# shenyunhang/JTSM

Measured on AMD Instinct MI355X. Metric: images/sec training, R50-FPN JTSM panoptic, 2x1024x1024, 1/2/4/8 GPU, higher is better.
Workload: dtype bf16x3; 1 GPU; BASELINE configs[2]: JTSM panoptic R50-FPN, 2 x 3x1024x1024 per GPU, 2000 proposals + 1024 superpixels per image; MIL + 4 OICR + 2 mask heads + sem-seg; fwd + bwd + gradient exchange + SGD; 100% of proposals jittered copies of 40 rectangles per image; global_batch=2, parallelism=dp1, foreground_rois_last_step=281

## Files before the change

### include/jtsm_hip.h

```cpp
#ifndef JTSM_HIP_H_
#define JTSM_HIP_H_

#include <stddef.h>
#include <stdint.h>

#ifdef __cplusplus
extern "C" {
#endif

#define JTSM_OK 0
#define JTSM_EINVAL (-1)
#define JTSM_ELAUNCH (-2)
#define JTSM_ENODEV (-3)

#define JTSM_NCHW 0
#define JTSM_NHWC 1

const char* jtsm_last_error(void);
const char* jtsm_version(void);
int jtsm_device_count(void);

void* jtsm_event_create(void);
int jtsm_event_record(void* event, void* stream);
int jtsm_event_elapsed_ms(void* start, void* stop, float* ms);
// ... 103 lines not shown
  int batch, in_h, in_w, in_c;
  int out_c;
  int kernel_h, kernel_w;
  int stride, pad, dilation;
} jtsm_conv_shape;

int jtsm_conv_out_size(const jtsm_conv_shape* s, int* out_h, int* out_w);
size_t jtsm_conv_workspace_bytes(const jtsm_conv_shape* s, int backward_data);
int jtsm_conv_plan(const jtsm_conv_shape* s, int role, int has_kscale, int* kernel, int* tile_m,
                   int* tile_n, int* splits);

int jtsm_conv2d_forward_f32(const float* x, const float* w, float* y, const jtsm_conv_shape* s,
                            const float* scale, const float* bias, const float* residual,
                            int relu, void* workspace, size_t workspace_bytes, void* stream);
int jtsm_conv2d_backward_data_f32(const float* dy, const float* w, float* dx,
                                  const jtsm_conv_shape* s, const float* kscale,
                                  const float* accumulate, const float* relu_mask, void* workspace,
                                  size_t workspace_bytes, void* stream);
int jtsm_conv2d_backward_weight_f32(const float* dy, const float* x, float* dw,
                                    const jtsm_conv_shape* s, const float* row_scale, int zero_dw,
                                    void* stream);

int jtsm_split_bf16_f32(const float* src, uint16_t* hi, uint16_t* lo, long n, void* stream);
int jtsm_split_bf16_paired_f32(const float* src, uint16_t* planes, long rows, int k, void* stream);
int jtsm_split_bf16_transposed_f32(const float* w, const float* row_scale, uint16_t* hi, uint16_t* lo,
                                   int out_c, int taps, int in_c, void* stream);
int jtsm_split_bf16_multi_f32(const void* table, int entries, long blocks, int transposed, void* stream);
int jtsm_conv_bf16x3_eligible(const jtsm_conv_shape* s, int role);
int jtsm_conv_bf16x3_plan(const jtsm_conv_shape* s, int role, int* wm, int* wn, int* tm, int* tn, int* nbuf,
                          int* splits);
int jtsm_conv2d_forward_bf16x3(const uint16_t* x_hi, const uint16_t* x_lo, const uint16_t* w_hi,
                               const uint16_t* w_lo, float* y, uint16_t* y_hi, uint16_t* y_lo,
                               const jtsm_conv_shape* s, const float* scale, const float* bias,
                               const float* residual, int relu, void* workspace, size_t workspace_bytes,
                               void* stream);
int jtsm_conv2d_backward_data_bf16x3(const uint16_t* dy_hi, const uint16_t* dy_lo, const uint16_t* wt_hi,
                                     const uint16_t* wt_lo, float* dx, uint16_t* dx_hi, uint16_t* dx_lo,
                                     const jtsm_conv_shape* s, const float* accumulate,
                                     const float* relu_mask, void* workspace, size_t workspace_bytes,
                                     void* stream);
size_t jtsm_conv_bf16x3_wgrad_workspace_bytes(const jtsm_conv_shape* s);
int jtsm_conv2d_backward_weight_bf16x3(const uint16_t* dy_hi, const uint16_t* dy_lo, const uint16_t* x_hi,
                                       const uint16_t* x_lo, float* dw, const jtsm_conv_shape* s,
                                       const float* row_scale, int zero_dw, void* workspace,
                                       size_t workspace_bytes, void* stream);

int jtsm_split_f16_f32(const float* src, uint16_t* h, long n, int shift, void* stream);
int jtsm_split_f16_transposed_f32(const float* w, const float* row_scale, uint16_t* h, int out_c, int taps, int in_c,
                                  void* stream);
int jtsm_conv2d_forward_f16(const uint16_t* x_h, const uint16_t* w_h, float* y, uint16_t* y_h,
                            const jtsm_conv_shape* s, const float* scale, const float* bias,
                            const float* residual, int relu, void* workspace, size_t workspace_bytes,
                            void* stream);
int jtsm_conv2d_backward_data_f16(const uint16_t* dy_h, const uint16_t* wt_h, float* dx, uint16_t* dx_h,
                                  const jtsm_conv_shape* s, const float* accumulate, const float* relu_mask,
                                  int grad_shift, void* workspace, size_t workspace_bytes, void* stream);
int jtsm_conv2d_backward_weight_f16(const uint16_t* dy_h, const uint16_t* x_h, float* dw, const jtsm_conv_shape* s,
                                    const float* row_scale, int zero_dw, int grad_shift, void* workspace,
                                    size_t workspace_bytes, void* stream);
int jtsm_conv_transpose2x2_forward_bf16x3(const uint16_t* x_hi, const uint16_t* x_lo, const uint16_t* wt_hi,
                                          const uint16_t* wt_lo, float* y, uint16_t* y_hi, uint16_t* y_lo, int batch,
                                          int h, int w, int in_c, int out_c, const float* bias, int relu, void* stream);
int jtsm_conv_transpose2x2_forward_f16(const uint16_t* x_h, const uint16_t* wt_h, float* y, uint16_t* y_h, int batch,
                                       int h, int w, int in_c, int out_c, const float* bias, int relu, void* stream);
size_t jtsm_conv_transpose2x2_workspace_bytes(int batch, int h, int w, int in_c, int out_c);
int jtsm_conv_transpose2x2_backward_data_bf16x3(const uint16_t* g_hi, const uint16_t* g_lo, const uint16_t* w_hi,
                                                const uint16_t* w_lo, float* dx, uint16_t* dx_hi, uint16_t* dx_lo,
                                                int batch, int h, int w, int in_c, int out_c, const float* relu_mask,
                                                const uint16_t* gate_plane, void* workspace, size_t workspace_bytes,
                                                void* stream);
int jtsm_conv_transpose2x2_backward_data_f16(const uint16_t* g_h, const uint16_t* w_h, float* dx, uint16_t* dx_h,
                                             int batch, int h, int w, int in_c, int out_c, const float* relu_mask,
                                             const uint16_t* gate_plane, int grad_shift, void* workspace,
                                             size_t workspace_bytes, void* stream);
int jtsm_conv2d_backward_data_ex_bf16x3(const uint16_t* dy_hi, const uint16_t* dy_lo, const uint16_t* wt_hi,
                                        const uint16_t* wt_lo, float* dx, uint16_t* dx_hi, uint16_t* dx_lo,
                                        const jtsm_conv_shape* s, const float* row_scale, const float* accumulate,
                                        const float* relu_mask, const uint16_t* gate_plane, void* workspace,
                                        size_t workspace_bytes, void* stream);
int jtsm_conv2d_backward_data_ex_f16(const uint16_t* dy_h, const uint16_t* wt_h, float* dx, uint16_t* dx_h,
                                     const jtsm_conv_shape* s, const float* row_scale, const float* accumulate,
                                     const float* relu_mask, const uint16_t* gate_plane, int grad_shift, void* workspace,
                                     size_t workspace_bytes, void* stream);

int jtsm_conv2d_forward_res16_f16(const uint16_t* x_h, const uint16_t* w_h, float* y, uint16_t* y_h,
                                  const jtsm_conv_shape* s, const float* scale, const float* bias,
                                  const uint16_t* residual_h, int relu, void* workspace, size_t workspace_bytes,
                                  void* stream);
int jtsm_conv2d_backward_data_acc16_f16(const uint16_t* dy_h, const uint16_t* wt_h, float* dx, uint16_t* dx_h,
                                        const jtsm_conv_shape* s, const float* row_scale, const uint16_t* accumulate_h,
                                        const uint16_t* gate_plane, int grad_shift, void* workspace,
                                        size_t workspace_bytes, void* stream);

int jtsm_conv_bf16x3_colsum_rows(const jtsm_conv_shape* s, int role);
int jtsm_conv2d_backward_data_colsum_bf16x3(const uint16_t* dy_hi, const uint16_t* dy_lo, const uint16_t* wt_hi,
                                            const uint16_t* wt_lo, float* dx, uint16_t* dx_hi, uint16_t* dx_lo,
                                            const jtsm_conv_shape* s, const float* row_scale, const float* accumulate,
                                            const float* relu_mask, const uint16_t* gate_plane, float* colsum,
                                            void* workspace, size_t workspace_bytes, void* stream);
int jtsm_conv2d_backward_data_colsum_f16(const uint16_t* dy_h, const uint16_t* wt_h, float* dx, uint16_t* dx_h,
                                         const jtsm_conv_shape* s, const float* row_scale, const float* accumulate,
                                         const float* relu_mask, const uint16_t* gate_plane, int grad_shift, float* colsum,
                                         void* workspace, size_t workspace_bytes, void* stream);
int jtsm_conv_transpose2x2_backward_data_colsum_bf16x3(const uint16_t* g_hi, const uint16_t* g_lo, const uint16_t* w_hi,
                                                       const uint16_t* w_lo, float* dx, uint16_t* dx_hi, uint16_t* dx_lo,
                                                       int batch, int h, int w, int in_c, int out_c,
                                                       const float* relu_mask, const uint16_t* gate_plane, float* colsum,
                                                       void* workspace, size_t workspace_bytes, void* stream);
int jtsm_conv_transpose2x2_backward_data_colsum_f16(const uint16_t* g_h, const uint16_t* w_h, float* dx, uint16_t* dx_h,
                                                    int batch, int h, int w, int in_c, int out_c, const float* relu_mask,
                                                    const uint16_t* gate_plane, int grad_shift, float* colsum,
                                                    void* workspace, size_t workspace_bytes, void* stream);
int jtsm_relu_backward_split_scaled_f32(const float* dy, const float* y, float scale, float* g, uint16_t* g_hi,
                                        uint16_t* g_lo, long n, int shift, void* stream);
int jtsm_split_rowscale_f32(const float* src, const float* row_scale, long rows, int cols, uint16_t* hi, uint16_t* lo,
                            int shift, void* stream);
int jtsm_dropout_split_f32(const float* x, float* y, uint16_t* y_hi, uint16_t* y_lo, long n, float p,
                           unsigned long long seed, void* stream);
int jtsm_channel_sum_planes(const uint16_t* hi, const uint16_t* lo, float* out, long rows, int C, int shift,
                            void* workspace, size_t workspace_bytes, void* stream);
int jtsm_channel_sum_planes_multi(const uint16_t* const* hi, const uint16_t* const* lo, float* const* outs,
                                  const long* rows, int count, int C, int shift, void* workspace,
                                  size_t workspace_bytes, void* stream);
size_t jtsm_conv_bf16x3_wgrad_bias_workspace_bytes(const jtsm_conv_shape* s);
int jtsm_conv2d_backward_weight_bias_bf16x3(const uint16_t* dy_hi, const uint16_t* dy_lo, const uint16_t* x_hi,
                                            const uint16_t* x_lo, float* dw, float* db, const jtsm_conv_shape* s,
                                            const float* row_scale, int zero_dw, void* workspace,
                                            size_t workspace_bytes, void* stream);
int jtsm_conv2d_backward_weight_bias_f16(const uint16_t* dy_h, const uint16_t* x_h, float* dw, float* db,
                                         const jtsm_conv_shape* s, const float* row_scale, int zero_dw, int grad_shift,
                                         void* workspace, size_t workspace_bytes, void* stream);
size_t jtsm_conv_bf16x3_wgrad_group_workspace_bytes(const jtsm_conv_shape* s, int n);
int jtsm_conv_bf16x3_wgrad_group_plan(const jtsm_conv_shape* s, int n, int* tile, int* splits);
int jtsm_conv2d_backward_weight_group_bf16x3(int n, const uint16_t* const* dy_hi, const uint16_t* const* dy_lo,
                                             const uint16_t* const* x_hi, const uint16_t* const* x_lo,
                                             float* const* dw, const float* const* row_scale,
                                             const jtsm_conv_shape* s, void* workspace, size_t workspace_bytes,
                                             void* stream);
int jtsm_conv2d_backward_weight_group_f16(int n, const uint16_t* const* dy_h, const uint16_t* const* x_h,
                                          float* const* dw, const float* const* row_scale, const jtsm_conv_shape* s,
                                          int grad_shift, void* workspace, size_t workspace_bytes, void* stream);
int jtsm_relu_backward_split_f16(const float* dy, const float* y, float* g, uint16_t* g_h, long n, int shift,
                                 void* stream);

int jtsm_relu_backward_split_f32(const float* dy, const float* y, float* g, uint16_t* g_hi, uint16_t* g_lo,
                                 long n, void* stream);
int jtsm_relu_backward_f32(const float* dy, const float* y, float* g, long n, void* stream);
int jtsm_channel_sum_f32(const float* g, float* out, long rows, int C, void* stream);
int jtsm_colsum_fold_f32(const float* const* parts, const int* rows, int n, int width, float* out, void* stream);
size_t jtsm_channel_sum_workspace_bytes(long rows, int C);
int jtsm_channel_sum_ws_f32(const float* g, float* out, long rows, int C, void* workspace, size_t workspace_bytes,
                            void* stream);
int jtsm_sgd_momentum_multi_f32(const void* table, int entries, long blocks, int first_step, void* stream);


int jtsm_maxpool3x3s2_forward_f32(const float* x, float* y, int N, int H, int W, int C, void* stream);
int jtsm_maxpool3x3s2_backward_f32(const float* x, const float* gy, float* gx, int N, int H, int W,
                                   int C, void* stream);
int jtsm_maxpool2x2_forward_f32(const float* x, float* y, int N, int H, int W, int C, int stride, void* stream);
int jtsm_maxpool2x2_backward_f32(const float* x, const float* gy, float* gx, int N, int H, int W, int C,
                                 int stride, void* stream);
int jtsm_upsample2_add_f32(const float* top, const float* lateral, float* out, uint16_t* out_hi, uint16_t* out_lo,
                           int N, int H, int W, int C, void* stream);
int jtsm_sum_tensors_f32(const float* const* inputs, int n, long numel, float* out, uint16_t* out_hi, uint16_t* out_lo,
                         void* stream);
int jtsm_sum2x2_f32(const float* g, float* out, int N, int Ht, int Wt, int C, void* stream);
int jtsm_subsample2_f32(const float* src, float* dst, int N, int H, int W, int C, int scatter,
                        void* stream);


size_t jtsm_mil_workspace_bytes(int nbags, int max_bag_rows, int nc);
int jtsm_mil_forward_f32(const float* cls_logits, const float* det_logits, int ld, int nc,
                         const int32_t* bag_offsets, int nbags, int max_bag_rows,
                         const float* labels, int mean_loss, float* scores, float* img_probs,
                         float* loss, void* workspace, void* stream);
int jtsm_mil_backward_f32(const float* cls_logits, const float* det_logits, int ld, int nc,
                          const int32_t* bag_offsets, int nbags, int max_bag_rows,
                          const float* upstream, float* d_cls, float* d_det, int ld_grad,
                          const void* workspace, void* stream);

size_t jtsm_oicr_workspace_bytes(void);
int jtsm_oicr_forward_f32(const float* cls_logits, int ld_cls, int num_cls, const float* box_deltas,
                          int ld_box, const int32_t* labels, const float* weights,
                          const float* proposals, const float* gt_boxes, int R, float* losses,
                          void* workspace, void* stream);
int jtsm_oicr_backward_f32(const float* cls_logits, int ld_cls, int num_cls, const float* box_deltas,
                           int ld_box, const int32_t* labels, const float* weights,
                           const float* proposals, const float* gt_boxes, int R, const float* losses,
                           const float* up_cls, const float* up_box, float* d_cls, int ld_dcls,
                           float* d_box, int ld_dbox, void* stream);


int jtsm_rect_mask_targets_f32(const float* rois, const float* rects, uint8_t* out, int N, int side, int H, int W,
                               float erode, void* stream);
int jtsm_sp_mask_targets_f32(const float* rois, const int32_t* oh_row, const int32_t* img_of, const int32_t* oh_labels,
                             int L, const int32_t* superpixels, uint8_t* out, int N, int side, int H, int W,
                             void* stream);
int jtsm_paste_crop_targets_f32(const float* probs, const float* rois, uint8_t* out, int N, int M, int side, int H,
                                int W, float threshold, void* stream);
int jtsm_near_targets_f32(const float* proposals, const int32_t* bag_offsets, int B, int R, const int32_t* labels,
                          int bg_label, const float* pgt_box, const int32_t* counts, int Gmax, int top_k,
                          int32_t* near_rows, int32_t* matched_near, void* stream);

int jtsm_pooler_rois_levels_f32(const float* const* boxes, const int* counts, int B, int min_level, int max_level,
                                float canonical_box_size, float canonical_level, float* rois, int32_t* level,
                                void* stream);
int jtsm_roi_scale_f32(const int32_t* argmax, int bins, int C, const float* const* objectness, const int* counts, int B,
                       float* out, void* stream);
size_t jtsm_image_labels_workspace_bytes(int B);
int jtsm_image_labels(const int64_t* const* gt_classes, const int* counts, int B, int num_classes, const void* sem_seg,
                      int sem_elem_bytes, long pixels, int num_stuff, int stuff_offset, float* oh_things,
                      int32_t* things_cls, int32_t* things_cnt, float* oh_stuff, int32_t* stuff_cls, int32_t* stuff_cnt,
                      void* workspace, void* stream);

int jtsm_fg_compact(const int32_t* labels, int bg_label, const int32_t* bag_offsets, int B, int R, const float* boxes,
                    const int32_t* matched, int32_t* fg_rows, float* fg_boxes, int64_t* fg_classes, int32_t* fg_img,
                    int32_t* fg_matched, float* fg_rois, int64_t* counts, void* stream);

size_t jtsm_mask_bce_workspace_bytes(void);
int jtsm_mask_bce_forward_f32(const float* logits, int ld, int num_classes, const int64_t* gt_classes,
                              const uint8_t* target, int N, int side, float* out, void* workspace,
                              void* stream);
int jtsm_mask_bce_backward_f32(const float* logits, int ld, int num_classes, const int64_t* gt_classes,
                               const uint8_t* target, int N, int side, const float* upstream,
                               float* dlogits, void* stream);


int jtsm_roi_align_forward_level_f32(const float* input, const float* rois,
                                     const int32_t* roi_level, int level, float* output, int B,
                                     int C, int H, int W, int M, float spatial_scale, int pooled_h,
                                     int pooled_w, int sampling_ratio, int aligned, void* stream);
int jtsm_roi_align_backward_level_f32(const float* grad, const float* rois,
                                      const int32_t* roi_level, int level, float* grad_input, int B,
                                      int C, int H, int W, int M, float spatial_scale, int pooled_h,
                                      int pooled_w, int sampling_ratio, int aligned, void* stream);
int jtsm_roi_align_rotated_forward_level_f32(const float* input, const float* rois, const int32_t* roi_level,
                                             int level, float* output, int B, int C, int H, int W, int M,
                                             float spatial_scale, int pooled_h, int pooled_w, int sampling_ratio,
                                             void* stream);
int jtsm_roi_align_rotated_backward_level_f32(const float* grad, const float* rois, const int32_t* roi_level,
                                              int level, float* grad_input, int B, int C, int H, int W, int M,
                                              float spatial_scale, int pooled_h, int pooled_w, int sampling_ratio,
                                              int accumulate, void* stream);
size_t jtsm_roi_align_backward_levels_workspace_bytes(const int* H, const int* W, int nlevels, int B, int C, int M);
int jtsm_roi_align_backward_levels_f32(const float* grad, const float* rois, const int32_t* roi_level,
                                       float* const* grad_inputs, const int* H, const int* W, const float* scales,
                                       int nlevels, int B, int C, int M, int pooled_h, int pooled_w, int sampling_ratio,
                                       int aligned, int accumulate, void* workspace, size_t workspace_bytes,
                                       void* stream);
int jtsm_moi_pool_forward_level_f32(const float* input, const float* rois, const int32_t* roi_level,
                                    int level, const int32_t* oh_labels, const int32_t* superpixels,
                                    float* output, int32_t* argmax, void* workspace, int B, int C,
                                    int H, int W, int M, int L, int Hs, int Ws, float spatial_scale,
                                    int pooled_h, int pooled_w, void* stream);
int jtsm_moi_pool_backward_level_f32(const float* grad, const float* rois, const int32_t* roi_level,
                                     int level, const int32_t* argmax, float* grad_input, int B, int C,
                                     int H, int W, int M, int pooled_h, int pooled_w, void* stream);


size_t jtsm_group_norm_workspace_bytes(int N, long HW, int C);
int jtsm_group_norm_forward_f32(const float* x, const float* gamma, const float* beta, float* y,
                                float* mean, float* rstd, void* workspace, int N, long HW, int C, int G,
                                float eps, int relu, void* stream);
int jtsm_group_norm_backward_f32(const float* x, const float* dy, const float* gamma, const float* beta,
                                 const float* mean, const float* rstd, float* dx, uint16_t* dx_hi,
                                 uint16_t* dx_lo, float* dgamma, float* dbeta, void* workspace, int N, long HW,
                                 int C, int G, int relu, void* stream);
int jtsm_upsample_bilinear2x_forward_f32(const float* x, float* y, uint16_t* y_hi, uint16_t* y_lo, int N, int H,
                                         int W, int C, void* stream);
int jtsm_upsample_bilinear2x_backward_f32(const float* gy, float* gx, int N, int H, int W, int C,
                                          void* stream);


size_t jtsm_semseg_ce_workspace_bytes(int N, int Hs, int Ws, int S);
int jtsm_semseg_ce_forward_f32(const float* logits, int ld, int C, const int64_t* target, float* out,
                               void* workspace, int N, int Hs, int Ws, int S, long ignore_index,
                               void* stream);
int jtsm_semseg_ce_backward_f32(const float* logits, int ld, int C, const int64_t* target,
                                const float* fwd_out, const float* upstream, float* dlogits,
                                const void* workspace, int N, int Hs, int Ws, int S, long ignore_index,
                                void* stream);


int jtsm_row_lse_f32(const float* logits, int ld, int ncls, int R, float* lse, void* stream);
int jtsm_mine_top1_f32(const float* scores, int ld, const float* lse, const float* proposals,
                       const float* deltas, int ld_deltas, const int32_t* bag_offsets,
                       const int32_t* classes, const int32_t* counts, int B, int Gmax,
                       const float* img_probs, int nprob, int32_t* out_idx, float* out_box,
                       float* out_score, float* out_weight, void* stream);
size_t jtsm_paint_sem_seg_workspace_bytes(int B);
int jtsm_paint_sem_seg(const float* boxes, const int32_t* classes, const float* scores, const int32_t* counts,
                       int B, int G, int class_base, int H, int W, float erode, int64_t* out, void* workspace,
                       void* stream);
int jtsm_paint_sem_seg_evidence(const int32_t* target_idx, const int32_t* bag_offsets, const int32_t* oh_labels, int L,
                                const int32_t* superpixels, const int32_t* classes, const float* scores,
                                const int32_t* counts, int B, int G, int class_base, int H, int W, int64_t* out,
                                void* workspace, void* stream);
int jtsm_match_label_f32(const float* proposals, const int32_t* bag_offsets, int B, int R,
                         const float* pgt_box, const int32_t* classes, const int32_t* counts,
                         const float* pgt_weight, const float* pgt_score, int Gmax, float iou_thresh,
                         int bg_label, int32_t* labels, int32_t* matched, float* gt_boxes,
                         float* gt_weights, float* gt_scores, void* stream);


int jtsm_oicr_predict_f32(const float* const* logits, const float* const* deltas, int heads, int R, int C1, int Kb,
                          const float* proposals, const float* weights , float scale_clamp, float* probs,
// ... 44 lines not shown
```

### jtsm_amd/build.py

```python
import argparse
import glob
import os
import subprocess
import sys
from concurrent.futures import ThreadPoolExecutor

HERE = os.path.dirname(os.path.abspath(__file__))
CSRC = os.path.join(HERE, "csrc")
OBJ = os.path.join(HERE, "lib", "obj")
LIB = os.path.join(HERE, "lib", "libjtsm_hip.so")
HIPCC = os.environ.get("HIPCC", "/opt/rocm/bin/hipcc")
FLAGS = ["--offload-arch=gfx950", "-O3", "-std=c++17", "-fPIC", "-Wall", "-Wno-unused-function",
         "-fno-gpu-rdc"] + os.environ.get("JTSM_EXTRA_HIPCC_FLAGS", "").split()
FILE_FLAGS = {"semseg_ops.hip": ["-fno-slp-vectorize"]}


def _stale(target, deps):
    if not os.path.isfile(target):
        return True
    t = os.path.getmtime(target)
    return any(os.path.getmtime(d) > t for d in deps)


def build(force=False, verbose=False, jobs=4):
    os.makedirs(OBJ, exist_ok=True)
    srcs = sorted(glob.glob(os.path.join(CSRC, "*.hip")))
    hdrs = sorted(glob.glob(os.path.join(CSRC, "*.h"))) + [
        os.path.join(HERE, "..", "include", "jtsm_hip.h")]
    todo, objs = [], []
    for s in srcs:
        o = os.path.join(OBJ, os.path.basename(s)[:-4] + ".o")
        objs.append(o)
        if force or _stale(o, [s, os.path.abspath(__file__)] + hdrs):
            todo.append((s, o))

    def cc(job):
        s, o = job
        cmd = [HIPCC] + FLAGS + FILE_FLAGS.get(os.path.basename(s), []) + ["-c", s, "-o", o]
        if verbose:
            print(" ".join(cmd), flush=True)
        r = subprocess.run(cmd, stdout=subprocess.PIPE, stderr=subprocess.STDOUT, text=True)
        return s, r.returncode, r.stdout

    if todo:
        with ThreadPoolExecutor(max_workers=jobs) as ex:
            for s, rc, out in ex.map(cc, todo):
                if out.strip() and (verbose or rc):
                    print(out, file=sys.stderr)
                if rc:
                    raise RuntimeError("hipcc failed on %s" % s)
    if todo or force or _stale(LIB, objs):
        cmd = [HIPCC, "--offload-arch=gfx950", "-shared", "-fPIC", "-o", LIB] + objs
        if verbose:
            print(" ".join(cmd), flush=True)
        subprocess.check_call(cmd)
    return LIB


if __name__ == "__main__":
    ap = argparse.ArgumentParser()
    ap.add_argument("--force", action="store_true")
    ap.add_argument("-v", "--verbose", action="store_true")
    a = ap.parse_args()
    print(build(force=a.force, verbose=a.verbose))
```

### jtsm_amd/layers/conv.py

```python
import ctypes as C
import os

import torch
from torch.autograd import Function
from torch.autograd.function import once_differentiable

from .. import _lib as L
from . import grad_fan

CL = torch.channels_last

LAUNCH_LOG = None
SEGMENT = "heads"


def set_segment(name):
    global SEGMENT
    SEGMENT = name


MATH = os.environ.get("JTSM_CONV_MATH", "bf16x3")
_MODES = ("f32", "bf16x3", "f16")
GRAD_SHIFT = int(os.environ.get("JTSM_F16_GRAD_SHIFT", "12"))
BIAS_IN_WGRAD = os.environ.get("JTSM_BIAS_IN_WGRAD", "1") != "0"


def planes_mode():
    return MATH != "f32"


def set_math(mode):
    global MATH
    if mode not in _MODES:
        raise ValueError("conv math must be one of %r, got %r" % (_MODES, mode))
    if mode != MATH:
        _drop_planes()
    MATH = mode


def _planes_buf(n, device):
    n8 = max((n + 7) // 8 * 8, 64)
    if MATH == "f16":
        return torch.empty(n8, dtype=torch.int16, device=device)
    return torch.empty(2 * n8, dtype=torch.int16, device=device)


def _hl(buf):
    if buf is None:
        return None, None
    p = buf.data_ptr()
    if MATH == "f16":
        return p, None
    if getattr(buf, "_paired", False):
        return p, p + 64
    return p, p + buf.numel()


W_PAIRED = os.environ.get("JTSM_W_PAIRED", "1") != "0"


def _paired_ok(w, transposed):
    if not W_PAIRED or MATH != "bf16x3" or w.numel() == 0:
        return 0
    k = w.numel() // w.shape[1 if transposed else 0]
    return k if k % 32 == 0 else 0


def _split(t, grad=False):
    flat = t.permute(0, 2, 3, 1) if t.dim() == 4 else t
    if not flat.is_contiguous():
        raise RuntimeError("split_bf16: tensor must be channels_last (4-d) or contiguous")
    buf = _planes_buf(t.numel(), t.device)
    hi, lo = _hl(buf)
    L.note_bytes((6.0 if MATH == "f16" else 8.0) * t.numel())
    if MATH == "f16":
        L.check(L.lib().jtsm_split_f16_f32(L.ptr(t), hi, t.numel(), GRAD_SHIFT if grad else 0, L.stream()), "split_f16")
        return buf
    L.check(L.lib().jtsm_split_bf16_f32(L.ptr(t), hi, lo, t.numel(), L.stream()), "split_bf16")
    return buf


def split_bf16(t):
    buf = _split(t)
    n8 = buf.numel() // 2
    return buf[:t.numel()], buf[n8:n8 + t.numel()]


def _split_paired(w):
    k = _paired_ok(w, False)
    buf = _planes_buf(w.numel(), w.device)
    buf._paired = True
    L.note_bytes(8.0 * w.numel())
    L.check(L.lib().jtsm_split_bf16_paired_f32(L.ptr(w), L.ptr(buf), w.numel() // k, k, L.stream()),
            "split_bf16_paired")
    return buf


def _split_transposed_into(buf, w, row_scale, paired=True):
    o, i, kh, kw = w.shape
    if paired and _paired_ok(w, True):
        buf._paired = True
    hi, lo = _hl(buf)
    if MATH == "f16":
        L.check(L.lib().jtsm_split_f16_transposed_f32(L.ptr(w), L.ptr(row_scale), hi, o, kh * kw, i, L.stream()),
                "split_f16_transposed")
    else:
        L.check(L.lib().jtsm_split_bf16_transposed_f32(L.ptr(w), L.ptr(row_scale), hi, lo, o, kh * kw, i, L.stream()),
                "split_bf16_transposed")
    return buf


def _split_transposed(w, row_scale=None, paired=True):
    return _split_transposed_into(_planes_buf(w.numel(), w.device), w, row_scale, paired)


def split_bf16_transposed(w, row_scale=None):
    buf = _split_transposed(w, row_scale, paired=False)
    n8 = buf.numel() // 2
    return buf[:w.numel()], buf[n8:n8 + w.numel()]


_PLANES = {}
_PLANES_MAX_BYTES = 16 << 30
_planes_bytes = 0


CLEAR_HOOKS = []


def planes_clear():
    global _planes_bytes
    _PLANES.clear()
    _planes_bytes = 0
    for hook in CLEAR_HOOKS:
        hook()
    refresh_weight_planes()


def _drop_planes():
    global _planes_bytes
    _PLANES.clear()
    _planes_bytes = 0
    _WPLANES.clear()
    _WTABLES.clear()


def planes_put(t, buf):
    global _planes_bytes
    if _planes_bytes > _PLANES_MAX_BYTES:
        _PLANES.clear()
        _planes_bytes = 0
    _PLANES[(t.data_ptr(), t.numel())] = (t.detach(), t._version, buf)
    _planes_bytes += 8 * t.numel()


def planes_forget(t):
    _PLANES.pop((t.data_ptr(), t.numel()), None)


def planes_of(t, grad=False):
    e = _PLANES.get((t.data_ptr(), t.numel()))
    if e is not None and e[1] == t._version:
        return e[2]
    buf = _split(t, grad)
    planes_put(t, buf)
    return buf


class _WEntry(object):
    __slots__ = ("w", "scale", "transposed", "buf", "version")


_WPLANES = {}
_WTABLES = {}


def _cacheable_weight(w):
    base = w._base if w._base is not None else w
    return isinstance(base, torch.nn.Parameter) and (w.dim() != 4 or w.permute(0, 2, 3, 1).is_contiguous())


def _weight_planes(w, transposed=False, scale=None):
    if not _cacheable_weight(w):
        if transposed:
            return _split_transposed(w, scale)
        return _split_paired(w) if _paired_ok(w, False) else _split(w)
    key = (w.data_ptr(), w.numel(), transposed, scale.data_ptr() if scale is not None else 0)
    e = _WPLANES.get(key)
    if e is not None and e.version == w._version:
        return e.buf
    if e is None:
        if len(_WPLANES) >= 2048:
            _WPLANES.clear()
            _WTABLES.clear()
        e = _WEntry()
        e.w, e.scale, e.transposed = w.detach(), scale, transposed
        e.buf = _planes_buf(w.numel(), w.device)
        e.buf._paired = bool(_paired_ok(w, transposed))
        _WPLANES[key] = e
    hi, lo = _hl(e.buf)
    lib = L.lib()
    if transposed:
        _split_transposed_into(e.buf, w, scale)
    elif e.buf._paired:
        L.check(lib.jtsm_split_bf16_paired_f32(L.ptr(w), hi, w.shape[0], w.numel() // w.shape[0], L.stream()),
                "split_bf16_paired")
    elif MATH == "f16":
        L.check(lib.jtsm_split_f16_f32(L.ptr(w), hi, w.numel(), 0, L.stream()), "split_f16")
    else:
        L.check(lib.jtsm_split_bf16_f32(L.ptr(w), hi, lo, w.numel(), L.stream()), "split_bf16")
    e.version = w._version
    return e.buf


def refresh_weight_planes():
    if MATH == "f32" or not _WPLANES:
        return
    for transposed in (False, True):
        stale = [(k, e) for k, e in _WPLANES.items() if e.transposed == transposed and e.version != e.w._version]
        if not stale:
            continue
        tkey = (transposed, tuple(k for k, _ in stale))
        tab = _WTABLES.get(tkey)
        if tab is None:
            rows, blocks = [], 0
            for _, e in stale:
                hi = e.buf.data_ptr()
                lo = 0 if MATH == "f16" else hi + e.buf.numel()
                paired = getattr(e.buf, "_paired", False)
                if paired:
                    lo = hi + 64
                if transposed:
                    o, i, kh, kw = e.w.shape
                    nb = ((i + 31) // 32) * ((o + 31) // 32) * kh * kw
                    rows.append([e.w.data_ptr(), hi, lo, e.scale.data_ptr() if e.scale is not None else 0, blocks, o,
                                 kh * kw, i])
                else:
                    nb = (e.w.numel() + 2047) // 2048
                    rows.append([e.w.data_ptr(), hi, lo, 0, blocks, e.w.numel(), 0,
                                 e.w.numel() // e.w.shape[0] if paired else 0])
                blocks += nb
            dev = stale[0][1].w.device
            tab = (torch.tensor(rows, dtype=torch.int64).to(dev), blocks)
            if len(_WTABLES) > 8:
                _WTABLES.clear()
            _WTABLES[tkey] = tab
        L.note_bytes((6.0 if MATH == "f16" else 8.0) * sum(e.w.numel() for _, e in stale))
        L.check(L.lib().jtsm_split_bf16_multi_f32(L.ptr(tab[0]), len(stale), tab[1], int(transposed), L.stream()),
                "split_bf16_multi")
        for _, e in stale:
            e.version = e.w._version


GRAD_SLOTS = {}


def grad_slot(w, params=None):
    if not GRAD_SLOTS or w is None:
        return None
    key = (w.data_ptr(), w.numel())
    e = GRAD_SLOTS.get(key)
    if e is None:
        return None
    p = e.param()
    if p is None or e.owner() is None or p.data_ptr() != key[0]:
        GRAD_SLOTS.pop(key, None)
        return None
    if p.grad is not None or e.written:
        return None
    e.written = True
    return e.view


class _Plan(object):
    __slots__ = ("s", "ref", "oh", "ow", "flops", "desc", "ws", "x3", "wgrad_big")


_PLANS = {}


def _plan(x_shape, w_shape, stride, pad, dil):
    key = (tuple(x_shape), tuple(w_shape), stride, pad, dil)
    p = _PLANS.get(key)
    if p is None:
        if len(_PLANS) >= 8192:
            _PLANS.clear()
        lib = L.lib()
        p = _Plan()
        p.wgrad_big = None
        p.s = _shape(x_shape, w_shape, stride, pad, dil)
        p.ref = C.byref(p.s)
        p.oh, p.ow = out_hw(p.s)
        p.flops = _flops(p.s)
        p.desc = _desc(p.s)
        p.x3 = tuple(bool(lib.jtsm_conv_bf16x3_eligible(p.ref, r)) and p.s.batch > 0 for r in range(3))
        p.ws = (lib.jtsm_conv_workspace_bytes(p.ref, 0), lib.jtsm_conv_workspace_bytes(p.ref, 1),
                lib.jtsm_conv_bf16x3_wgrad_workspace_bytes(p.ref), lib.jtsm_conv_bf16x3_wgrad_bias_workspace_bytes(p.ref))
        _PLANS[key] = p
    return p


_SCRATCH = {}


def _scratch(nbytes, device):
    if nbytes == 0:
        return None
    key = (device, L.stream())
    buf = _SCRATCH.get(key)
    if buf is None or buf.numel() < nbytes:
        buf = _SCRATCH[key] = torch.empty(int(nbytes * 1.25) + 256, dtype=torch.uint8, device=device)
    return buf


_ON_SIDE_STREAM = [False]


def _x3_variant(s, role):
    if LAUNCH_LOG is None:
        return None
    v = [C.c_int() for _ in range(6)]
    L.check(L.lib().jtsm_conv_bf16x3_plan(C.byref(s), role, *[C.byref(x) for x in v]), "conv_bf16x3_plan")
    wm, wn, tm, tn, nbuf, splits = [x.value for x in v]
    np_ = ",1" if MATH == "f16" else ""
    if role == 2:
        if nbuf == 0:
            return _Variant("igemm_x3_wgrad_halo_kernel" + ("<1>" if MATH == "f16" else ""), splits)
        return _Variant("igemm_x3_wgrad_kernel<%d,%d,%d,%d,%d%s>" % (wm, wn, tm, tn, nbuf, np_), splits)
    if nbuf == 0:
        return _Variant("igemm_x3_halo_kernel<%s,%d,%d,%d,%d,%d%s>" % (_ROLE_NAME[role], 16 if wm == 4 else 8, wm, wn,
                                                                       tn, 21 if wm == 4 else 12, np_), splits)
    return _Variant("igemm_x3_kernel<%s,%d,%d,%d,%d,%d%s>" % (_ROLE_NAME[role], wm, wn, tm, tn, nbuf, np_), splits)


class _Variant(str):
    def __new__(cls, name, splits=1):
        o = str.__new__(cls, name)
        o.splits = splits
        return o


class LaunchSpan(object):
    __slots__ = ("a", "mid", "b")

    def __init__(self):
        lib = L.lib()
        self.a, self.mid, self.b = lib.jtsm_event_create(), lib.jtsm_event_create(), lib.jtsm_event_create()

    def _ms(self, x, y):
        out = C.c_float()
        return out.value if L.lib().jtsm_event_elapsed_ms(x, y, C.byref(out)) == 0 else None

    def kernel_ms(self):
        ms = self._ms(self.a, self.mid)
        return ms if ms is not None else self._ms(self.a, self.b)

    def call_ms(self):
        return self._ms(self.a, self.b)

    def __del__(self):
        try:
            lib = L.lib()
            for e in (self.a, self.mid, self.b):
                lib.jtsm_event_destroy(e)
        except Exception:
            pass


def _timed(variant, flops, call, shape=None, extra_elems=0, out_elems=0, planes=False, fp32_out=True):
    if LAUNCH_LOG is None:
        return call()
    splits = getattr(variant, "splits", 1)
    finish_bytes = 0.0
    if splits > 1:
        plane_b = (2.0 if MATH == "f16" else 4.0) if planes else 0.0
        finish_bytes = out_elems * (4.0 * splits + (4.0 if fp32_out else 0.0) + plane_b) + 4.0 * extra_elems
    if shape is not None and extra_elems and splits <= 1:
        shape = shape[:-1] + (shape[-1] + 4.0 * extra_elems,)
    lib = L.lib()
    span = LaunchSpan()
    st = L.stream()
    lib.jtsm_event_record(span.a, st)
    lib.jtsm_conv_set_mid_event(span.mid)
    rc = call()
    lib.jtsm_conv_set_mid_event(None)
    lib.jtsm_event_record(span.b, st)
    if variant is not None:
        variant.segment = SEGMENT
    LAUNCH_LOG.append((variant, flops, span, shape, finish_bytes))
    return rc


_ROLE_NAME = ("FWD", "DGRAD", "WGRAD")


def _numel(t):
    return 0 if t is None else t.numel()


def _variant(s, role, has_kscale=False):
    if LAUNCH_LOG is None:
        return None
    k, bm, bn, sp = C.c_int(), C.c_int(), C.c_int(), C.c_int()
    L.check(L.lib().jtsm_conv_plan(C.byref(s), role, int(has_kscale), C.byref(k), C.byref(bm), C.byref(bn),
# ... 963 lines not shown
```

### jtsm_amd/solver/build.py

```python
import struct

import torch

from .. import _lib as L


def _f32_bits(x):
    return struct.unpack("<I", struct.pack("<f", float(x)))[0]


class SGD(torch.optim.Optimizer):

    def __init__(self, params, lr, momentum=0.0, weight_decay=0.0):
        if momentum <= 0.0:
            raise ValueError("jtsm_amd SGD is the momentum form (the reference trains with momentum 0.9)")
        super().__init__(params, dict(lr=lr, momentum=momentum, weight_decay=weight_decay))

    def attach_early_heads(self, model, prefixes=("roi_heads.", "sem_seg_head.")):
        import os
        import weakref
        from ..layers import conv
        if os.environ.get("JTSM_EARLY_STEP", "1") == "0":
            return self
        self._early_ids = {id(p) for n, p in model.named_parameters() if p.requires_grad and n.startswith(tuple(prefixes))}
        self._stepped = set()
        ref = weakref.ref(self)

        def hook():
            opt = ref()
            if opt is not None:
                opt._early_step()
        self._early_hook = hook
        conv.HEADS_DONE_HOOKS.append(hook)
        return self

    def detach_early_heads(self):
        from ..layers import conv
        hook = self.__dict__.pop("_early_hook", None)
        if hook in conv.HEADS_DONE_HOOKS:
            conv.HEADS_DONE_HOOKS.remove(hook)
        self._early_ids = set()

    @torch.no_grad()
    def _early_step(self):
        from ..layers import conv
        ids = getattr(self, "_early_ids", None)
        if not ids or not conv.WGRAD_STREAM or self._stepped:
            return
        todo = []
        for group in self.param_groups:
            for p in group["params"]:
                if id(p) in ids and p.grad is not None:
                    if not p.is_cuda or getattr(p, "_post_accumulate_grad_hooks", None):
                        return
                    todo.append(p)
        conv.flush_deferred_weight_gradients()
        todo = [p for g in self.param_groups for p in g["params"] if id(p) in ids and p.grad is not None]
        if not todo or not conv.queue_side_stream_join():
            return
        device = todo[0].device
        side = conv._wgrad_side_stream(device)
        side.wait_stream(torch.cuda.current_stream(device))
        for s in conv.PRODUCER_STREAMS:
            if s is not side and s.device == device:
                side.wait_stream(s)
        with torch.cuda.stream(side):
            for p in todo:
                p.grad.record_stream(side)
            self._apply(only=ids, staging="_staging_early")
            conv.refresh_weight_planes()
        self._stepped = {id(p) for p in todo}

    @torch.no_grad()
    def step(self, closure=None):
        loss = None
        if closure is not None:
            with torch.enable_grad():
                loss = closure()
        self._apply(skip=getattr(self, "_stepped", None) or None)
        if getattr(self, "_stepped", None):
            self._stepped = set()
        return loss

    def _apply(self, only=None, skip=None, staging="_staging"):
        rows, blocks, device, keep, touched = [], 0, None, [], []
        for group in self.param_groups:
            lr, wd, mu = _f32_bits(group["lr"]), _f32_bits(group["weight_decay"]), _f32_bits(group["momentum"])
            for p in group["params"]:
                g = p.grad
                if g is None or (only is not None and id(p) not in only) or (skip is not None and id(p) in skip):
                    continue
                if not p.is_cuda or p.dtype != torch.float32:
                    raise RuntimeError("jtsm_amd SGD updates float32 parameters on the HIP device only")
                st = self.state[p]
                if "momentum_buffer" not in st:
                    st["momentum_buffer"] = torch.zeros_like(p, memory_format=torch.preserve_format)
                buf = st["momentum_buffer"]
                if g.stride() != p.stride() or buf.stride() != p.stride():
                    g = torch.empty_like(p, memory_format=torch.preserve_format).copy_(g)
                    keep.append(g)
                n = p.numel()
                rows.append([p.data_ptr(), g.data_ptr(), buf.data_ptr(), n, blocks, lr, wd, mu])
                touched.append(p)
                touched.append(buf)
                blocks += (n + 1023) // 1024
                device = p.device
        if rows:
            nwords = len(rows) * 8
            st = self.__dict__.setdefault(staging, {"host": [None, None], "dev": None, "turn": 0,
                                                    "copied": [None, None]})
            if st["dev"] is None or st["dev"].numel() < nwords or st["dev"].device != device:
                st["host"] = [torch.empty(nwords, dtype=torch.int64).pin_memory() for _ in range(2)]
                st["dev"] = torch.empty(nwords, dtype=torch.int64, device=device)
                st["copied"] = [None, None]
            st["turn"] ^= 1
            host = st["host"][st["turn"]]
            if st["copied"][st["turn"]] is not None:
                st["copied"][st["turn"]].synchronize()
            host[:nwords].copy_(torch.tensor(rows, dtype=torch.int64).view(-1))
            table = st["dev"][:nwords]
            table.copy_(host[:nwords], non_blocking=True)
            ev = torch.cuda.Event()
            ev.record()
            st["copied"][st["turn"]] = ev
            L.note_bytes(20.0 * sum(r[3] for r in rows))
            L.check(L.lib().jtsm_sgd_momentum_multi_f32(L.ptr(table), len(rows), blocks, 0, L.stream()),
                    "sgd_momentum_multi")
            torch.autograd.graph.increment_version(touched)


def build_optimizer(cfg, model):
    norm_types = (torch.nn.BatchNorm2d, torch.nn.GroupNorm, torch.nn.LayerNorm, torch.nn.SyncBatchNorm)
    groups, seen = [], set()
    for module in model.modules():
        for name, p in module.named_parameters(recurse=False):
            if not p.requires_grad or p in seen:
                continue
            seen.add(p)
            lr, wd = cfg.SOLVER.BASE_LR, cfg.SOLVER.WEIGHT_DECAY
            if isinstance(module, norm_types):
                wd = cfg.SOLVER.WEIGHT_DECAY_NORM
            elif name == "bias":
                lr = cfg.SOLVER.BASE_LR * cfg.SOLVER.BIAS_LR_FACTOR
                wd = cfg.SOLVER.WEIGHT_DECAY_BIAS
            groups.append({"params": [p], "lr": lr, "weight_decay": wd})
    return SGD(groups, cfg.SOLVER.BASE_LR, momentum=cfg.SOLVER.MOMENTUM)
```

Measured before the change: 98.54 images/sec.

## Fuse SGD update with bf16 hi/lo weight plane regeneration

```diff
diff --git a/include/jtsm_hip.h b/include/jtsm_hip.h
--- a/include/jtsm_hip.h
+++ b/include/jtsm_hip.h
@@ -279,6 +279,7 @@
 int jtsm_channel_sum_ws_f32(const float* g, float* out, long rows, int C, void* workspace, size_t workspace_bytes,
                             void* stream);
 int jtsm_sgd_momentum_multi_f32(const void* table, int entries, long blocks, int first_step, void* stream);
+int jtsm_sgd_momentum_planes_multi_f32(const void* table, int entries, long blocks, int first_step, void* stream);
 
 
 int jtsm_maxpool3x3s2_forward_f32(const float* x, float* y, int N, int H, int W, int C, void* stream);
diff --git a/jtsm_amd/build.py b/jtsm_amd/build.py
--- a/jtsm_amd/build.py
+++ b/jtsm_amd/build.py
@@ -12,7 +12,7 @@
 HIPCC = os.environ.get("HIPCC", "/opt/rocm/bin/hipcc")
 FLAGS = ["--offload-arch=gfx950", "-O3", "-std=c++17", "-fPIC", "-Wall", "-Wno-unused-function",
          "-fno-gpu-rdc"] + os.environ.get("JTSM_EXTRA_HIPCC_FLAGS", "").split()
-FILE_FLAGS = {"semseg_ops.hip": ["-fno-slp-vectorize"]}
+FILE_FLAGS = {"semseg_ops.hip": ["-fno-slp-vectorize"], "sgd_planes.hip": ["-fno-slp-vectorize"]}
 
 
 def _stale(target, deps):
diff --git a/jtsm_amd/csrc/sgd_planes.hip b/jtsm_amd/csrc/sgd_planes.hip
--- /dev/null
+++ b/jtsm_amd/csrc/sgd_planes.hip
@@ -0,0 +1,208 @@
+#include <cstdint>
+
+#include "common.h"
+
+namespace jtsm {
+namespace {
+
+typedef __bf16 sp_bf16x4 __attribute__((ext_vector_type(4)));
+typedef __bf16 sp_bf16x8 __attribute__((ext_vector_type(8)));
+
+struct SgdPlanesEntry {
+  float* p; const float* g; float* buf; long n; long first_block; long lr; long wd; long mu;
+  __bf16* s_hi; __bf16* s_lo;
+  __bf16* t_hi; __bf16* t_lo;
+  const float* row_scale;
+  long out_c; long taps; long in_c;
+};
+
+constexpr int kTile = 64;
+
+__device__ __forceinline__ float word_f32(long w) { return __int_as_float((int)w); }
+
+__device__ __forceinline__ bool sp_paired(const __bf16* hi, const __bf16* lo) { return lo - hi == 32; }
+__device__ __forceinline__ size_t sp_paired_index(size_t row, size_t k, size_t K) {
+  return row * 2 * K + (k >> 5) * 64 + (k & 31);
+}
+
+__device__ __forceinline__ void sgd1(float& p, float g, float& b, float lr, float wd, float mu, int first) {
+  const float d = __fmaf_rn(p, wd, g);
+  b = first ? d : __fmaf_rn(b, mu, d);
+  p = __fmaf_rn(-b, lr, p);
+}
+
+__device__ __forceinline__ void split1(float v, __bf16& h, __bf16& l) {
+  h = (__bf16)v;
+  l = (__bf16)(v - (float)h);
+}
+
+__device__ __forceinline__ void straight1(const SgdPlanesEntry& t, size_t i, size_t K, float v) {
+  if (sp_paired(t.s_hi, t.s_lo)) {
+    const size_t row = i / K, o = sp_paired_index(row, i - row * K, K);
+    split1(v, t.s_hi[o], t.s_hi[o + 32]);
+  } else {
+    split1(v, t.s_hi[i], t.s_lo[i]);
+  }
+}
+__device__ __forceinline__ void straight4(const SgdPlanesEntry& t, size_t i, size_t K, const float (&v)[4]) {
+  sp_bf16x4 h, l;
+#pragma unroll
+  for (int e = 0; e < 4; ++e) {
+    __bf16 hh, ll;
+    split1(v[e], hh, ll);
+    h[e] = hh; l[e] = ll;
+  }
+  if (sp_paired(t.s_hi, t.s_lo)) {
+    const size_t row = i / K, o = sp_paired_index(row, i - row * K, K);
+    *reinterpret_cast<sp_bf16x4*>(t.s_hi + o) = h;
+    *reinterpret_cast<sp_bf16x4*>(t.s_hi + o + 32) = l;
+  } else {
+    *reinterpret_cast<sp_bf16x4*>(t.s_hi + i) = h;
+    *reinterpret_cast<sp_bf16x4*>(t.s_lo + i) = l;
+  }
+}
+
+__global__ __launch_bounds__(256) void sgd_planes_multi_kernel(const SgdPlanesEntry* __restrict__ tab, int nent,
+                                                               int first_step) {
+  __shared__ float tile[kTile][kTile + 1];
+  int lo = 0, hi = nent - 1;
+  while (lo < hi) {
+    const int mid = (lo + hi + 1) >> 1;
+    if (tab[mid].first_block <= (long)blockIdx.x) lo = mid; else hi = mid - 1;
+  }
+  const SgdPlanesEntry t = tab[lo];
+  const float lr = word_f32(t.lr), wd = word_f32(t.wd), mu = word_f32(t.mu);
+  const int Cout = (int)t.out_c, taps = (int)t.taps, Cin = (int)t.in_c;
+  const size_t K = (size_t)taps * Cin;
+  const bool aligned = ((((uintptr_t)t.p | (uintptr_t)t.g | (uintptr_t)t.buf) & 15) == 0);
+
+  if (!t.t_hi) {
+    const long base = ((long)blockIdx.x - t.first_block) * 1024 + threadIdx.x * 4;
+    if (base >= t.n) return;
+    if (base + 4 <= t.n && aligned && (K & 3) == 0) {
+      const float4 p4 = *reinterpret_cast<const float4*>(t.p + base), g4 = *reinterpret_cast<const float4*>(t.g + base);
+      const float4 b4 = first_step ? make_float4(0.f, 0.f, 0.f, 0.f) : *reinterpret_cast<const float4*>(t.buf + base);
+      float p[4] = {p4.x, p4.y, p4.z, p4.w}, b[4] = {b4.x, b4.y, b4.z, b4.w};
+      const float g[4] = {g4.x, g4.y, g4.z, g4.w};
+#pragma unroll
+      for (int e = 0; e < 4; ++e) sgd1(p[e], g[e], b[e], lr, wd, mu, first_step);
+      *reinterpret_cast<float4*>(t.buf + base) = make_float4(b[0], b[1], b[2], b[3]);
+      *reinterpret_cast<float4*>(t.p + base) = make_float4(p[0], p[1], p[2], p[3]);
+      if (t.s_hi) straight4(t, (size_t)base, K, p);
+    } else {
+      for (long i = base; i < t.n && i < base + 4; ++i) {
+        float p = t.p[i], b = first_step ? 0.f : t.buf[i];
+        sgd1(p, t.g[i], b, lr, wd, mu, first_step);
+        t.buf[i] = b;
+        t.p[i] = p;
+        if (t.s_hi) straight1(t, (size_t)i, K, p);
+      }
+    }
+    return;
+  }
+
+  const int nx = (Cin + kTile - 1) / kTile, ny = (Cout + kTile - 1) / kTile;
+  long r = (long)blockIdx.x - t.first_block;
+  const int bx = (int)(r % nx); r /= nx;
+  const int by = (int)(r % ny);
+  const int tap = (int)(r / ny);
+  if (tap >= taps) return;
+  const int ci0 = bx * kTile, co0 = by * kTile;
+  if (aligned && (Cin & 3) == 0) {
+    const int c = (threadIdx.x & 15) * 4, r0 = threadIdx.x >> 4;
+#pragma unroll
+    for (int j = 0; j < kTile / 16; ++j) {
+      const int row = r0 + 16 * j, co = co0 + row, ci = ci0 + c;
+      if (co < Cout && ci < Cin) {
+        const size_t off = ((size_t)co * taps + tap) * Cin + ci;
+        const float4 p4 = *reinterpret_cast<const float4*>(t.p + off), g4 = *reinterpret_cast<const float4*>(t.g + off);
+        const float4 b4 = first_step ? make_float4(0.f, 0.f, 0.f, 0.f) : *reinterpret_cast<const float4*>(t.buf + off);
+        float p[4] = {p4.x, p4.y, p4.z, p4.w}, b[4] = {b4.x, b4.y, b4.z, b4.w};
+        const float g[4] = {g4.x, g4.y, g4.z, g4.w};
+#pragma unroll
+        for (int e = 0; e < 4; ++e) sgd1(p[e], g[e], b[e], lr, wd, mu, first_step);
+        *reinterpret_cast<float4*>(t.buf + off) = make_float4(b[0], b[1], b[2], b[3]);
+        *reinterpret_cast<float4*>(t.p + off) = make_float4(p[0], p[1], p[2], p[3]);
+        if (t.s_hi) straight4(t, off, K, p);
+        if (t.row_scale) {
+          const float sc = t.row_scale[co];
+#pragma unroll
+          for (int e = 0; e < 4; ++e) p[e] *= sc;
+        }
+#pragma unroll
+        for (int e = 0; e < 4; ++e) tile[row][c + e] = p[e];
+      }
+    }
+  } else {
+    for (int idx = threadIdx.x; idx < kTile * kTile; idx += 256) {
+      const int row = idx >> 6, col = idx & (kTile - 1), co = co0 + row, ci = ci0 + col;
+      if (co < Cout && ci < Cin) {
+        const size_t off = ((size_t)co * taps + tap) * Cin + ci;
+        float p = t.p[off], b = first_step ? 0.f : t.buf[off];
+        sgd1(p, t.g[off], b, lr, wd, mu, first_step);
+        t.buf[off] = b;
+        t.p[off] = p;
+        if (t.s_hi) straight1(t, off, K, p);
+        tile[row][col] = t.row_scale ? p * t.row_scale[co] : p;
+      }
+    }
+  }
+  __syncthreads();
+  const size_t Kt = (size_t)taps * Cout;
+  const bool paired = sp_paired(t.t_hi, t.t_lo);
+  if ((Cout & 7) == 0 && ((((uintptr_t)t.t_hi | (uintptr_t)t.t_lo) & 15) == 0)) {
+    for (int pc = threadIdx.x; pc < kTile * kTile / 8; pc += 256) {
+      const int row = pc >> 3, c = (pc & 7) * 8, ci = ci0 + row, co = co0 + c;
+      if (ci < Cin && co < Cout) {
+        sp_bf16x8 h, l;
+#pragma unroll
+        for (int e = 0; e < 8; ++e) {
+          __bf16 hh, ll;
+          split1(tile[c + e][row], hh, ll);
+          h[e] = hh; l[e] = ll;
+        }
+        if (paired) {
+          const size_t o = sp_paired_index(ci, (size_t)tap * Cout + co, Kt);
+          *reinterpret_cast<sp_bf16x8*>(t.t_hi + o) = h;
+          *reinterpret_cast<sp_bf16x8*>(t.t_hi + o + 32) = l;
+        } else {
+          const size_t o = ((size_t)ci * taps + tap) * Cout + co;
+          *reinterpret_cast<sp_bf16x8*>(t.t_hi + o) = h;
+          *reinterpret_cast<sp_bf16x8*>(t.t_lo + o) = l;
+        }
+      }
+    }
+  } else {
+    for (int idx = threadIdx.x; idx < kTile * kTile; idx += 256) {
+      const int row = idx >> 6, c = idx & (kTile - 1), ci = ci0 + row, co = co0 + c;
+      if (ci < Cin && co < Cout) {
+        if (paired) {
+          const size_t o = sp_paired_index(ci, (size_t)tap * Cout + co, Kt);
+          split1(tile[c][row], t.t_hi[o], t.t_hi[o + 32]);
+        } else {
+          const size_t o = ((size_t)ci * taps + tap) * Cout + co;
+          split1(tile[c][row], t.t_hi[o], t.t_lo[o]);
+        }
+      }
+    }
+  }
+}
+
+}
+}
+
+using namespace jtsm;
+
+extern "C" {
+
+int jtsm_sgd_momentum_planes_multi_f32(const void* table, int entries, long blocks, int first_step, void* stream) {
+  JTSM_REQUIRE(entries >= 0 && blocks >= 0 && blocks < 2147483647L, "sgd_planes_multi: bad sizes");
+  if (entries == 0 || blocks == 0) return JTSM_OK;
+  JTSM_REQUIRE(table && ((uintptr_t)table & 15) == 0, "sgd_planes_multi: table must be a 16-byte aligned device pointer");
+  hipLaunchKernelGGL(sgd_planes_multi_kernel, dim3((unsigned)blocks), dim3(256), 0, as_stream(stream),
+                     reinterpret_cast<const SgdPlanesEntry*>(table), entries, first_step);
+  JTSM_CHECK_LAUNCH("sgd_planes_multi");
+  return JTSM_OK;
+}
+
+}
diff --git a/jtsm_amd/layers/conv.py b/jtsm_amd/layers/conv.py
--- a/jtsm_amd/layers/conv.py
+++ b/jtsm_amd/layers/conv.py
@@ -143,6 +143,7 @@
     _planes_bytes = 0
     _WPLANES.clear()
     _WTABLES.clear()
+    _WBYMEM.clear()
 
 
 def planes_put(t, buf):
@@ -173,6 +174,7 @@
 
 _WPLANES = {}
 _WTABLES = {}
+_WBYMEM = {}
 
 
 def _cacheable_weight(w):
@@ -193,11 +195,13 @@
         if len(_WPLANES) >= 2048:
             _WPLANES.clear()
             _WTABLES.clear()
+            _WBYMEM.clear()
         e = _WEntry()
         e.w, e.scale, e.transposed = w.detach(), scale, transposed
         e.buf = _planes_buf(w.numel(), w.device)
         e.buf._paired = bool(_paired_ok(w, transposed))
         _WPLANES[key] = e
+        _WBYMEM.setdefault(key[:2], []).append(e)
     hi, lo = _hl(e.buf)
     lib = L.lib()
     if transposed:
@@ -250,6 +254,39 @@
                 "split_bf16_multi")
         for _, e in stale:
             e.version = e.w._version
+
+
+def fused_update_planes(p):
+    if MATH != "bf16x3":
+        return None
+    found = _WBYMEM.get((p.data_ptr(), p.numel()))
+    if not found or not (p.is_contiguous() or (p.dim() == 4 and p.is_contiguous(memory_format=CL))):
+        return None
+    straight = transposed = None
+    for e in found:
+        if e.transposed and transposed is None:
+            transposed = e
+        elif not e.transposed and straight is None:
+            straight = e
+    w = (transposed or straight).w
+    if w.dim() == 4:
+        out_c, in_c, taps = w.shape[0], w.shape[1], w.shape[2] * w.shape[3]
+    else:
+        out_c, in_c, taps = w.shape[0], w.numel() // max(w.shape[0], 1), 1
+    words = [0, 0, 0, 0, 0, out_c, taps, in_c]
+    if straight is not None:
+        if straight.w.shape[0] != out_c:
+            return None
+        words[0], words[1] = _hl(straight.buf)
+    if transposed is not None:
+        words[2], words[3] = _hl(transposed.buf)
+        words[4] = transposed.scale.data_ptr() if transposed.scale is not None else 0
+    return [e for e in (straight, transposed) if e is not None], words
+
+
+def planes_mark_fresh(entries):
+    for e in entries:
+        e.version = e.w._version
 
 
 GRAD_SLOTS = {}
diff --git a/jtsm_amd/solver/build.py b/jtsm_amd/solver/build.py
--- a/jtsm_amd/solver/build.py
+++ b/jtsm_amd/solver/build.py
@@ -1,8 +1,12 @@
+import os
 import struct
 
 import torch
 
 from .. import _lib as L
+
+
+FUSED_PLANES = os.environ.get("JTSM_SGD_FUSED_PLANES", "1") != "0"
 
 
 def _f32_bits(x):
@@ -17,7 +21,6 @@
         super().__init__(params, dict(lr=lr, momentum=momentum, weight_decay=weight_decay))
 
     def attach_early_heads(self, model, prefixes=("roi_heads.", "sem_seg_head.")):
-        import os
         import weakref
         from ..layers import conv
         if os.environ.get("JTSM_EARLY_STEP", "1") == "0":
@@ -83,7 +86,8 @@
         return loss
 
     def _apply(self, only=None, skip=None, staging="_staging"):
-        rows, blocks, device, keep, touched = [], 0, None, [], []
+        from ..layers import conv
+        rows, blocks, prows, pblocks, fresh, device, keep, touched = [], 0, [], 0, [], None, [], []
         for group in self.param_groups:
             lr, wd, mu = _f32_bits(group["lr"]), _f32_bits(group["weight_decay"]), _f32_bits(group["momentum"])
             for p in group["params"]:
@@ -100,13 +104,22 @@
                     g = torch.empty_like(p, memory_format=torch.preserve_format).copy_(g)
                     keep.append(g)
                 n = p.numel()
-                rows.append([p.data_ptr(), g.data_ptr(), buf.data_ptr(), n, blocks, lr, wd, mu])
+                planes = conv.fused_update_planes(p) if FUSED_PLANES else None
+                if planes is not None:
+                    entries, words = planes
+                    out_c, taps, in_c = words[5:]
+                    prows.append([p.data_ptr(), g.data_ptr(), buf.data_ptr(), n, pblocks, lr, wd, mu] + words)
+                    fresh.extend(entries)
+                    pblocks += ((in_c + 63) // 64) * ((out_c + 63) // 64) * taps if words[2] else (n + 1023) // 1024
+                else:
+                    rows.append([p.data_ptr(), g.data_ptr(), buf.data_ptr(), n, blocks, lr, wd, mu])
+                    blocks += (n + 1023) // 1024
                 touched.append(p)
                 touched.append(buf)
-                blocks += (n + 1023) // 1024
                 device = p.device
-        if rows:
-            nwords = len(rows) * 8
+        if rows or prows:
+            pwords = len(prows) * 16
+            nwords = pwords + len(rows) * 8
             st = self.__dict__.setdefault(staging, {"host": [None, None], "dev": None, "turn": 0,
                                                     "copied": [None, None]})
             if st["dev"] is None or st["dev"].numel() < nwords or st["dev"].device != device:
@@ -117,16 +130,25 @@
             host = st["host"][st["turn"]]
             if st["copied"][st["turn"]] is not None:
                 st["copied"][st["turn"]].synchronize()
-            host[:nwords].copy_(torch.tensor(rows, dtype=torch.int64).view(-1))
+            if prows:
+                host[:pwords].copy_(torch.tensor(prows, dtype=torch.int64).view(-1))
+            if rows:
+                host[pwords:nwords].copy_(torch.tensor(rows, dtype=torch.int64).view(-1))
             table = st["dev"][:nwords]
             table.copy_(host[:nwords], non_blocking=True)
             ev = torch.cuda.Event()
             ev.record()
             st["copied"][st["turn"]] = ev
-            L.note_bytes(20.0 * sum(r[3] for r in rows))
-            L.check(L.lib().jtsm_sgd_momentum_multi_f32(L.ptr(table), len(rows), blocks, 0, L.stream()),
-                    "sgd_momentum_multi")
+            if prows:
+                L.note_bytes(sum(r[3] * (20.0 + (4.0 if r[8] else 0.0) + (4.0 if r[10] else 0.0)) for r in prows))
+                L.check(L.lib().jtsm_sgd_momentum_planes_multi_f32(L.ptr(table), len(prows), pblocks, 0, L.stream()),
+                        "sgd_momentum_planes_multi")
+            if rows:
+                L.note_bytes(20.0 * sum(r[3] for r in rows))
+                L.check(L.lib().jtsm_sgd_momentum_multi_f32(L.ptr(table[pwords:]), len(rows), blocks, 0, L.stream()),
+                        "sgd_momentum_multi")
             torch.autograd.graph.increment_version(touched)
+            conv.planes_mark_fresh(fresh)
 
 
 def build_optimizer(cfg, model):
```

Result: no change. 99.22 images/sec (median of 6 runs) (+0.7%).
